# Jittor/JNeRF

Measured on NVIDIA H100. Metric: ngp_lego_train_rays_per_s, higher is better.
Workload: dtype f16

## Files before the change

include/ngp_b200.h:

```cpp
#ifndef NGP_B200_H
#define NGP_B200_H
#include <stdint.h>
#ifdef __cplusplus
extern "C" {
#endif

#define NGP_F32 0
#define NGP_F16 1
#define NGP_N_LEVELS 16
#define NGP_LEVEL_BYTES 32

const char* ngp_last_error(void);
int ngp_version(void);
int ngp_sm_count(void);
int ngp_debug_timeout_flag(void);

int ngp_hash_offsets(double aabb_scale, int n_levels, int base_resolution, int log2_hashmap_size,
                     uint32_t* offsets_out_host, double* per_level_scale_out);
int ngp_hash_level_table(void* stream, const uint32_t* offsets_host, int n_levels, uint32_t base_resolution,
                         float log2_per_level_scale, void* levels_dev);
int ngp_hash_level_table_primes(void* stream, const uint32_t* offsets_host, int n_levels, uint32_t base_resolution,
                                float log2_per_level_scale, void* levels_dev, uint32_t prime0, uint32_t prime1, uint32_t prime2);

int ngp_hash_fwd(void* stream, uint32_t n, const float* x, const void* grid, int dtype, const void* levels_dev, void* out);
// ... 59 lines not shown
                        const uint32_t* numsteps, uint32_t cascades, float* rgb_out, float* alpha_out);
int ngp_composite_loss_bwd(void* stream, uint32_t n_rays, uint32_t n_elements, const void* net_out, const float* coords,
                           const uint32_t* numsteps_in, const uint32_t* numsteps_compacted, const float* bg,
                           const float* target, float huber_delta, const float* density_grid_mean, uint32_t cascades,
                           float* rgb_out, float* loss_out, void* dnet_out, float reg_scale);

int ngp_render_workspace_bytes(uint32_t n_rays, uint32_t capacity, uint64_t* layout_out);
int ngp_render_init(void* stream, uint32_t n_rays, uint32_t capacity, void* workspace, float aabb_lo, float aabb_hi, const float* rays_o,
                    const float* rays_d, float cone_angle, float near_distance, uint32_t cascades, int const_dt, uint64_t rng_state,
                    uint64_t rng_inc, uint32_t jitter_tile, float* rgb_out, float* alpha_out, uint32_t* n_samples_out, uint32_t* n_alive_host);
int ngp_render_march_round(void* stream, uint32_t n_rays, uint32_t capacity, void* workspace, uint32_t n_alive, uint32_t k_steps, float aabb_lo,
                           float aabb_hi, const float* rays_o, const float* rays_d, const uint8_t* bitfield, float cone_angle, uint32_t cascades,
                           int const_dt);
int ngp_render_composite_round(void* stream, uint32_t n_rays, uint32_t capacity, void* workspace, uint32_t n_alive, uint32_t k_steps,
                               float min_transmittance, uint32_t cascades, float* rgb_out, float* alpha_out, uint32_t* n_samples_out,
                               uint32_t* n_alive_host);

int ngp_grid_mark_untrained(void* stream, uint32_t n_elements, float* grid, uint32_t n_images, const float* focal_lengths,
                            const float* xforms, int res_x, int res_y);
int ngp_grid_generate_samples(void* stream, uint32_t n_elements, uint64_t rng_state, uint64_t rng_inc, const uint32_t* step_dev,
                              float aabb_lo, float aabb_hi, const float* grid_in, float* positions_out, uint32_t* indices_out,
                              uint32_t n_cascades, float thresh);
int ngp_grid_splat(void* stream, uint32_t n, const uint32_t* indices, const void* mlp_out, int dtype, float* grid_tmp);
int ngp_grid_ema(void* stream, uint32_t n_elements, float decay, float* grid, const float* grid_tmp);
int ngp_grid_update_bitfield(void* stream, const float* grid, float* mean_out, uint8_t* bitfield, uint32_t cascades);

int ngp_adam_ema(void* stream, uint64_t n, void* param, int param_dtype, void* grad, int grad_dtype, float grad_scale,
                 float* m, float* v, float* master, float lr, float beta1, float beta2, float eps, uint32_t step,
                 float ema_decay, int zero_grad);
int ngp_train_sweep(void* stream, uint64_t n_entries, void* table, float* m, float* v, float* master, void* fx, const float* w_part,
                    uint32_t bwd_rows, void* w_density, float* wd_m, float* wd_v, float* wd_master, void* w_rgb, float* wr_m,
                    float* wr_v, float* wr_master, float lr, float beta1, float beta2, float eps, uint32_t step, float ema_decay);

int ngp_dp_exchange_step(void* stream, int world, int rank, uint64_t slice_len, uint32_t n_w, void* const* peer_table,
                         void* const* peer_table_grad, float* const* peer_w_grad, uint32_t* const* peer_flags, uint32_t epoch, float* m,
                         float* v, float* master, void* w_param, float* w_m, float* w_v, float* w_master, float grad_scale, float lr,
                         float beta1, float beta2, float eps, uint32_t step, float ema_decay);
int ngp_dp_exchange_wait(void* stream, int world, const uint32_t* my_flags, uint32_t epoch);
int ngp_ipc_export(const void* dev_ptr, uint8_t* handle64, uint64_t* offset);
int ngp_ipc_open(const uint8_t* handle64, uint64_t offset, void** dev_ptr);
int ngp_ipc_close(void* dev_ptr, uint64_t offset);

int ngp_raygen(void* stream, uint32_t n, const uint32_t* pix_index, uint32_t W, uint32_t H, const float* xforms,
               const float* focal, const float* principal, uint32_t* img_id_out, float* rays_o, float* rays_d);

int ngp_prepare_batch(void* stream, uint32_t n, const uint32_t* pix_index, uint32_t W, uint32_t H, const float* xforms,
                      const float* focal, const float* principal, const void* images_rgba, int image_is_u8, const float* bg,
// ... 30 lines not shown
```

jnerf_b200/csrc/grid_update.cu:

```cuda
#include "ngp_common.cuh"

namespace {

__global__ void mark_untrained_kernel(uint32_t n_elements, float* __restrict__ grid, uint32_t n_images, const float* __restrict__ focal,
                                      const float* __restrict__ xforms, float half_resx, float half_resy) {
    const uint32_t i = blockIdx.x * blockDim.x + threadIdx.x;
    if (i >= n_elements) return;
    const uint32_t level = i / NERF_GRID_N, pos_idx = i % NERF_GRID_N;
    const uint32_t x = morton3D_invert(pos_idx >> 0), y = morton3D_invert(pos_idx >> 1), z = morton3D_invert(pos_idx >> 2);
    const float sc = scalbnf(1.0f, (int)level);
    const float p[3] = {(((float)x + 0.5f) / NERF_GRIDSIZE - 0.5f) * sc + 0.5f, (((float)y + 0.5f) / NERF_GRIDSIZE - 0.5f) * sc + 0.5f,
                        (((float)z + 0.5f) / NERF_GRIDSIZE - 0.5f) * sc + 0.5f};
    const float voxel_radius = 0.5f * 1.73205080757f * sc / NERF_GRIDSIZE;
    int count = 0;
    for (uint32_t j = 0; j < n_images; ++j) {
        const float* m = xforms + 12 * j;
        const float pl[3] = {p[0] - __ldg(m + 9), p[1] - __ldg(m + 10), p[2] - __ldg(m + 11)};
        const float cx = pl[0] * __ldg(m + 0) + (pl[1] * __ldg(m + 1) + pl[2] * __ldg(m + 2));
        const float cy = pl[0] * __ldg(m + 3) + (pl[1] * __ldg(m + 4) + pl[2] * __ldg(m + 5));
        const float cz = pl[0] * __ldg(m + 6) + (pl[1] * __ldg(m + 7) + pl[2] * __ldg(m + 8));
        if (cz > 0.f) {
            if (fabsf(cx) - voxel_radius < cz / __ldg(focal + 2 * j) * half_resx && fabsf(cy) - voxel_radius < cz / __ldg(focal + 2 * j + 1) * half_resy) {
                count++;
                break;
// ... 26 lines not shown
                        (((float)z + r2) / NERF_GRIDSIZE - 0.5f) * sc + 0.5f};
    positions[3 * (size_t)i] = (p[0] - lo) / diag;
    positions[3 * (size_t)i + 1] = (p[1] - lo) / diag;
    positions[3 * (size_t)i + 2] = (p[2] - lo) / diag;
    indices[i] = idx;
}

template <typename T>
__global__ void splat_kernel(uint32_t n, const uint32_t* __restrict__ indices, const T* __restrict__ mlp_out, float* __restrict__ grid_tmp) {
    const uint32_t i = blockIdx.x * blockDim.x + threadIdx.x;
    if (i >= n) return;
    const float mlp = __expf((float)mlp_out[i]);
    const float thick = mlp * (1.73205080757f / 1024.0f);
    atomicMax(reinterpret_cast<uint32_t*>(grid_tmp) + indices[i], __float_as_uint(thick));
}

__global__ void ema_kernel(uint32_t n, float decay, float* __restrict__ grid, const float* __restrict__ grid_tmp) {
    const uint32_t i = blockIdx.x * blockDim.x + threadIdx.x;
    if (i >= n) return;
    const float prev = grid[i];
    grid[i] = (prev < 0.f) ? prev : fmaxf(prev * decay, grid_tmp[i]);
}

constexpr int MEAN_BLOCKS = 256;
__global__ void __launch_bounds__(256) mean_partial_kernel(const float* __restrict__ grid, float* __restrict__ partial) {
    __shared__ float s[256];
    float acc = 0.f;
    const uint32_t per_block = NERF_GRID_N / MEAN_BLOCKS;
    const float* g = grid + (size_t)blockIdx.x * per_block;
    for (uint32_t k = threadIdx.x; k < per_block; k += 256) acc += fmaxf(g[k], 0.f) / NERF_GRID_N;
    s[threadIdx.x] = acc;
    __syncthreads();
    for (int off = 128; off > 0; off >>= 1) {
        if ((int)threadIdx.x < off) s[threadIdx.x] += s[threadIdx.x + off];
        __syncthreads();
    }
    if (threadIdx.x == 0) partial[blockIdx.x] = s[0];
}
__global__ void __launch_bounds__(256) mean_final_kernel(const float* __restrict__ partial, float* __restrict__ mean) {
    __shared__ float s[256];
    s[threadIdx.x] = partial[threadIdx.x];
    __syncthreads();
    for (int off = 128; off > 0; off >>= 1) {
        if ((int)threadIdx.x < off) s[threadIdx.x] += s[threadIdx.x + off];
        __syncthreads();
    }
// ... 6 lines not shown
    const float m = *mean;
    const float thresh = 0.01f < m ? 0.01f : m;
    const float4 a = reinterpret_cast<const float4*>(grid)[2 * (size_t)i], b = reinterpret_cast<const float4*>(grid)[2 * (size_t)i + 1];
    uint8_t v = 0;
    v |= a.x > thresh ? 1 : 0; v |= a.y > thresh ? 2 : 0; v |= a.z > thresh ? 4 : 0; v |= a.w > thresh ? 8 : 0;
    v |= b.x > thresh ? 16 : 0; v |= b.y > thresh ? 32 : 0; v |= b.z > thresh ? 64 : 0; v |= b.w > thresh ? 128 : 0;
    bits[i] = v;
}
__global__ void bitfield_max_pool_kernel(uint32_t n, const uint8_t* __restrict__ prev, uint8_t* __restrict__ next) {
    const uint32_t i = blockIdx.x * blockDim.x + threadIdx.x;
    if (i >= n) return;
    const uint2 p = reinterpret_cast<const uint2*>(prev)[i];
    uint8_t bits = 0;
#pragma unroll
    for (int j = 0; j < 4; ++j) {
        bits |= ((p.x >> (8 * j)) & 0xFF) ? (uint8_t)(1 << j) : 0;
        bits |= ((p.y >> (8 * j)) & 0xFF) ? (uint8_t)(1 << (4 + j)) : 0;
    }
    const uint32_t x = morton3D_invert(i >> 0) + NERF_GRIDSIZE / 8, y = morton3D_invert(i >> 1) + NERF_GRIDSIZE / 8,
                   z = morton3D_invert(i >> 2) + NERF_GRIDSIZE / 8;
    next[morton3D(x, y, z)] |= bits;
}

float* g_mean_partial = nullptr;

}

extern "C" {

int ngp_grid_mark_untrained(void* stream, uint32_t n_elements, float* grid, uint32_t n_images, const float* focal_lengths, const float* xforms,
                            int res_x, int res_y) {
    if (n_elements == 0) return 0;
    mark_untrained_kernel<<<(n_elements + 127) / 128, 128, 0, (cudaStream_t)stream>>>(n_elements, grid, n_images, focal_lengths, xforms,
                                                                                     res_x * 0.5f, res_y * 0.5f);
    NGP_LAUNCH_CHECK();
    return 0;
}

int ngp_grid_generate_samples(void* stream, uint32_t n_elements, uint64_t rng_state, uint64_t rng_inc, const uint32_t* step_dev, float aabb_lo,
                              float aabb_hi, const float* grid_in, float* positions_out, uint32_t* indices_out, uint32_t n_cascades, float thresh) {
    if (n_elements == 0) return 0;
    generate_samples_kernel<<<(n_elements + 127) / 128, 128, 0, (cudaStream_t)stream>>>(n_elements, rng_state, rng_inc, step_dev, aabb_lo, aabb_hi,
                                                                                       grid_in, positions_out, indices_out, n_cascades, thresh);
    NGP_LAUNCH_CHECK();
    return 0;
}

int ngp_grid_splat(void* stream, uint32_t n, const uint32_t* indices, const void* mlp_out, int dtype, float* grid_tmp) {
    if (n == 0) return 0;
    if (dtype == 1) splat_kernel<__half><<<(n + 127) / 128, 128, 0, (cudaStream_t)stream>>>(n, indices, (const __half*)mlp_out, grid_tmp);
    else if (dtype == 0) splat_kernel<float><<<(n + 127) / 128, 128, 0, (cudaStream_t)stream>>>(n, indices, (const float*)mlp_out, grid_tmp);
    else NGP_REQUIRE(false, "ngp_grid_splat: bad dtype");
    NGP_LAUNCH_CHECK();
    return 0;
}

int ngp_grid_ema(void* stream, uint32_t n_elements, float decay, float* grid, const float* grid_tmp) {
    if (n_elements == 0) return 0;
    ema_kernel<<<(n_elements + 255) / 256, 256, 0, (cudaStream_t)stream>>>(n_elements, decay, grid, grid_tmp);
    NGP_LAUNCH_CHECK();
    return 0;
}

int ngp_grid_update_bitfield(void* stream, const float* grid, float* mean_out, uint8_t* bitfield, uint32_t cascades) {
    NGP_REQUIRE(cascades >= 1 && cascades <= 8, "ngp_grid_update_bitfield: cascades out of range");
    NGP_REQUIRE(((size_t)grid) % 16 == 0, "Can only reduce_sum on 16-byte aligned memory.");
    cudaStream_t s = (cudaStream_t)stream;
    if (!g_mean_partial) NGP_CHECK_CUDA(cudaMalloc(&g_mean_partial, MEAN_BLOCKS * sizeof(float)));
    mean_partial_kernel<<<MEAN_BLOCKS, 256, 0, s>>>(grid, g_mean_partial);
    mean_final_kernel<<<1, 256, 0, s>>>(g_mean_partial, mean_out);
    const uint32_t n = NERF_GRID_N / 8 * cascades;
    grid_to_bitfield_kernel<<<(n + 127) / 128, 128, 0, s>>>(n, grid, bitfield, mean_out);
    for (uint32_t level = 1; level < cascades; ++level) {
        bitfield_max_pool_kernel<<<(NERF_GRID_N / 64 + 127) / 128, 128, 0, s>>>(NERF_GRID_N / 64, bitfield + (size_t)NERF_GRID_N * (level - 1) / 8,
                                                                                bitfield + (size_t)NERF_GRID_N * level / 8);
    }
    NGP_LAUNCH_CHECK();
    return 0;
}

}
```

jnerf_b200/lib.py:

```python
import ctypes as C
import os

HERE = os.path.dirname(os.path.abspath(__file__))
LIB_PATH = os.environ.get("NGP_B200_LIB") or os.path.join(HERE, "libngp_b200.so")

_vp, _u32, _u64, _i64, _f32, _i32, _f64 = C.c_void_p, C.c_uint32, C.c_uint64, C.c_int64, C.c_float, C.c_int, C.c_double

SIGNATURES = {
    "ngp_last_error": (C.c_char_p, []),
    "ngp_version": (_i32, []),
    "ngp_sm_count": (_i32, []),
    "ngp_debug_timeout_flag": (_i32, []),
    "ngp_hash_offsets": (_i32, [_f64, _i32, _i32, _i32, _vp, _vp]),
    "ngp_hash_level_table": (_i32, [_vp, _vp, _i32, _u32, _f32, _vp]),
    "ngp_hash_level_table_primes": (_i32, [_vp, _vp, _i32, _u32, _f32, _vp, _u32, _u32, _u32]),
    "ngp_hash_fwd": (_i32, [_vp, _u32, _vp, _vp, _i32, _vp, _vp]),
    "ngp_hash_bwd": (_i32, [_vp, _u32, _vp, _vp, _i32, _vp, _vp, _u64]),
    "ngp_sh_fwd": (_i32, [_vp, _u32, _vp, _i32, _vp]),
    "ngp_mlp_fwd": (_i32, [_vp, _vp, _vp, _vp, _vp, _u32, _u32]),
    "ngp_mlp_bwd": (_i32, [_vp, _vp, _vp, _vp, _vp, _vp, _vp, _vp, _u32, _u32, _u32]),
    "ngp_mlp_bwd_dgrad": (_i32, [_vp, _vp, _vp, _vp, _vp, _vp, _u32, _u32]),
    "ngp_mlp_param_count": (_i32, [_u32]),
    "ngp_network_fwd": (_i32, [_vp, _u32, _vp, _vp, _vp, _vp, _vp, _vp, _vp, _vp]),
    "ngp_network_bwd": (_i32, [_vp, _u32, _vp, _vp, _vp, _vp, _vp, _vp, _vp, _vp, _vp, _vp]),
# ... 6 lines not shown
    "ngp_nerf_density": (_i32, [_vp, _u32, _vp, _vp, _vp]),
    "ngp_nerf_bwd": (_i32, [_vp, _u32, _vp, _vp, _vp, _vp, _vp, _vp]),
    "ngp_mesh_workspace_bytes": (_i32, [_u32, _u64, _u64, _vp]),
    "ngp_density_lattice": (_i32, [_vp, _u32, _vp, _vp, _vp, _vp]),
    "ngp_marching_cubes": (_i32, [_vp, _u32, _vp, _f32, _vp, _vp, _u64, _vp, _u64, _vp]),
    "ngp_mesh_largest_component": (_i32, [_vp, _u64, _u64, _vp, _vp, _vp, _vp, _vp, _vp]),
    "ngp_mesh_vertex_normals": (_i32, [_vp, _u64, _u64, _vp, _vp, _vp, _vp]),
    "ngp_mesh_smooth_workspace_bytes": (_i32, [_u32, _u32, _vp]),
    "ngp_mesh_smooth": (_i32, [_vp, _u32, _vp, _u32, _u32, _vp, _u64, _vp, _vp]),
    "ngp_render_workspace_bytes": (_i32, [_u32, _u32, _vp]),
    "ngp_render_init": (_i32, [_vp, _u32, _u32, _vp, _f32, _f32, _vp, _vp, _f32, _f32, _u32, _i32, _u64, _u64, _u32, _vp, _vp, _vp, _vp]),
    "ngp_render_march_round": (_i32, [_vp, _u32, _u32, _vp, _u32, _u32, _f32, _f32, _vp, _vp, _vp, _f32, _u32, _i32]),
    "ngp_render_composite_round": (_i32, [_vp, _u32, _u32, _vp, _u32, _u32, _f32, _u32, _vp, _vp, _vp, _vp]),
    "ngp_march_workspace_bytes": (_u64, [_u32]),
    "ngp_march": (_i32, [_vp, _u32, _f32, _f32, _u32, _vp, _vp, _vp, _f32, _f32, _u32, _i32, _u64, _u64, _vp, _vp, _vp, _vp, _vp]),
    "ngp_compact": (_i32, [_vp, _u32, _u32, _vp, _vp, _vp, _vp, _vp, _i32]),
    "ngp_composite_fwd": (_i32, [_vp, _u32, _vp, _i32, _vp, _vp, _vp, _vp, _u32, _vp]),
    "ngp_composite_bwd": (_i32, [_vp, _u32, _u32, _vp, _i32, _vp, _vp, _vp, _vp, _vp, _u32, _vp]),
    "ngp_composite_infer": (_i32, [_vp, _u32, _vp, _i32, _vp, _vp, _u32, _vp, _vp]),
    "ngp_composite_loss_bwd": (_i32, [_vp, _u32, _u32, _vp, _vp, _vp, _vp, _vp, _vp, _f32, _vp, _u32, _vp, _vp, _vp, _f32]),
    "ngp_grid_mark_untrained": (_i32, [_vp, _u32, _vp, _u32, _vp, _vp, _i32, _i32]),
    "ngp_grid_generate_samples": (_i32, [_vp, _u32, _u64, _u64, _vp, _f32, _f32, _vp, _vp, _vp, _u32, _f32]),
    "ngp_grid_splat": (_i32, [_vp, _u32, _vp, _vp, _i32, _vp]),
    "ngp_grid_ema": (_i32, [_vp, _u32, _f32, _vp, _vp]),
    "ngp_grid_update_bitfield": (_i32, [_vp, _vp, _vp, _vp, _u32]),
    "ngp_adam_ema": (_i32, [_vp, _u64, _vp, _i32, _vp, _i32, _f32, _vp, _vp, _vp, _f32, _f32, _f32, _f32, _u32, _f32, _i32]),
    "ngp_train_sweep": (_i32, [_vp, _u64, _vp, _vp, _vp, _vp, _vp, _vp, _u32, _vp, _vp, _vp, _vp, _vp, _vp, _vp, _vp, _f32, _f32, _f32, _f32, _u32,
                               _f32]),
    "ngp_train_sweep_dev": (_i32, [_vp, _u64, _vp, _vp, _vp, _vp, _vp, _vp, _u32, _vp, _vp, _vp, _vp, _vp, _vp, _vp, _vp, _vp]),
    "ngp_dp_exchange_step": (_i32, [_vp, _i32, _i32, _u64, _u32, _vp, _vp, _vp, _vp, _u32, _vp, _vp, _vp, _vp, _vp, _vp, _vp, _f32, _f32, _f32,
                                    _f32, _f32, _u32, _f32]),
    "ngp_dp_exchange_wait": (_i32, [_vp, _i32, _vp, _u32]),
    "ngp_ipc_export": (_i32, [_vp, _vp, _vp]),
    "ngp_ipc_open": (_i32, [_vp, _u64, _vp]),
    "ngp_ipc_close": (_i32, [_vp, _u64]),
    "ngp_raygen": (_i32, [_vp, _u32, _vp, _u32, _u32, _vp, _vp, _vp, _vp, _vp, _vp]),
    "ngp_prepare_batch": (_i32, [_vp, _u32, _vp, _u32, _u32, _vp, _vp, _vp, _vp, _i32, _vp, _vp, _vp, _vp, _vp]),
    "ngp_blend_target": (_i32, [_vp, _u32, _vp, _vp, _vp]),
    "ngp_step_state_bytes": (_u64, []),
    "ngp_step_state_set": (_i32, [_vp, _vp, _u64, _u64, _u32, _u32, _f32, _f32, _f32, _f32, _f32, _f32]),
    "ngp_step_state_tick": (_i32, [_vp, _vp, _u32, _f32, _f32, _f32, _f32, _f32, _f32]),
    "ngp_prepare_batch_dev": (_i32, [_vp, _u32, _vp, _vp, _u32, _u32, _u32, _vp, _vp, _vp, _vp, _i32, _vp, _vp, _vp, _vp, _vp]),
    "ngp_march_dev": (_i32, [_vp, _u32, _f32, _f32, _u32, _vp, _vp, _vp, _f32, _f32, _u32, _i32, _vp, _u32, _vp, _vp, _vp, _vp, _vp]),
    "ngp_adam_ema_dev": (_i32, [_vp, _u64, _vp, _i32, _vp, _i32, _vp, _vp, _vp, _vp, _i32]),
    "ngp_pcg32_seed": (None, [_u64, _u64, _vp]),
    "ngp_pcg32_advance": (None, [_vp, _i64]),
}

KERNELS_PER_CALL = {
    "ngp_hash_level_table": 1, "ngp_hash_level_table_primes": 1, "ngp_hash_fwd": 1, "ngp_hash_bwd": 1, "ngp_sh_fwd": 1, "ngp_mlp_fwd": 1, "ngp_mlp_bwd": 1, "ngp_mlp_bwd_dgrad": 1,
    "ngp_network_fwd": 1, "ngp_network_bwd": 1, "ngp_network_bwd_fx": 1, "ngp_train_sweep": 1, "ngp_train_sweep_dev": 1, "ngp_density_fwd": 1, "ngp_march": 3, "ngp_compact": 1, "ngp_composite_fwd": 1,
    "ngp_composite_bwd": 1, "ngp_composite_infer": 1, "ngp_composite_loss_bwd": 1, "ngp_grid_mark_untrained": 1,
    "ngp_grid_generate_samples": 1, "ngp_grid_splat": 1, "ngp_grid_ema": 1, "ngp_grid_update_bitfield": 7, "ngp_adam_ema": 1, "ngp_dp_exchange_step": 1, "ngp_dp_exchange_wait": 1, "ngp_raygen": 1, "ngp_prepare_batch": 1,
    "ngp_blend_target": 1, "ngp_step_state_set": 1, "ngp_step_state_tick": 1, "ngp_prepare_batch_dev": 1, "ngp_march_dev": 3, "ngp_adam_ema_dev": 1,
    "ngp_density_lattice": 1, "ngp_marching_cubes": 3, "ngp_mesh_largest_component": 18, "ngp_mesh_vertex_normals": 7,
    "ngp_render_init": 3, "ngp_render_march_round": 3, "ngp_render_composite_round": 3,
    "ngp_nerf_fwd": 1, "ngp_nerf_density": 1, "ngp_nerf_bwd": 3,
}
launch_count = 0
_lib = None


class NgpError(RuntimeError):
    pass


def load():
    global _lib
    if _lib is None:
        if not os.path.exists(LIB_PATH):
            raise NgpError(f"{LIB_PATH} is missing: build it with `python jnerf_b200/build.py` (nvcc, sm_90a). "
                           "There is no CPU fallback.")
        lib = C.CDLL(LIB_PATH)
        for name, (res, args) in SIGNATURES.items():
            fn = getattr(lib, name)
            fn.restype = res
# ... 14 lines not shown
```

jnerf_b200/ops.py:

```python
import numpy as np
import torch

from . import lib

F32, F16 = 0, 1


def _dt(t):
    if t.dtype == torch.float16:
        return F16
    if t.dtype == torch.float32:
        return F32
    raise TypeError(f"unsupported dtype {t.dtype}")


def _p(t):
    if t is None:
        return None
    assert t.is_cuda and t.is_contiguous(), "device-resident contiguous tensor required"
    return t.data_ptr()


_raw_stream, _raw_device = getattr(torch._C, "_cuda_getCurrentRawStream", None), getattr(torch._C, "_cuda_getDevice", None)

# ... 340 lines not shown
    if loss is None:
        loss = torch.empty(R, dtype=torch.float32, device=dev)
    lib.call("ngp_composite_loss_bwd", _stream(), R, net.shape[0], _p(net), _p(coords), _p(numsteps_in), _p(numsteps_c), _p(bg), _p(target),
             float(delta), _p(mean), cascades, _p(rgb), _p(loss), _p(dnet), float(reg_scale))
    return rgb, loss, dnet


def grid_mark_untrained(grid, focal, xforms, res):
    lib.call("ngp_grid_mark_untrained", _stream(), grid.numel(), _p(grid), xforms.shape[0], _p(focal), _p(xforms), int(res[0]), int(res[1]))


def grid_generate_samples(n, rng, step_dev, aabb, grid, n_cascades, thresh):
    pos = torch.empty((n, 3), dtype=torch.float32, device=grid.device)
    idx = torch.empty(n, dtype=torch.int32, device=grid.device)
    lib.call("ngp_grid_generate_samples", _stream(), n, int(rng[0]), int(rng[1]), _p(step_dev), float(aabb[0]), float(aabb[1]), _p(grid), _p(pos),
             _p(idx), n_cascades, float(thresh))
    return pos, idx


def grid_splat(indices, mlp_out, grid_tmp):
    lib.call("ngp_grid_splat", _stream(), indices.numel(), _p(indices), _p(mlp_out), _dt(mlp_out), _p(grid_tmp))


def grid_ema(grid, grid_tmp, decay=0.95):
    lib.call("ngp_grid_ema", _stream(), grid.numel(), float(decay), _p(grid), _p(grid_tmp))


def grid_update_bitfield(grid, mean, bitfield, cascades=5):
    lib.call("ngp_grid_update_bitfield", _stream(), _p(grid), _p(mean), _p(bitfield), cascades)


def adam_ema(param, grad, m, v, master, lr, step, beta1=0.9, beta2=0.99, eps=1e-15, ema_decay=0.95, grad_scale=1.0, zero_grad=True):
    lib.call("ngp_adam_ema", _stream(), param.numel(), _p(param), _dt(param), _p(grad), _dt(grad), float(grad_scale), _p(m), _p(v), _p(master),
             float(lr), float(beta1), float(beta2), float(eps), int(step), float(ema_decay), int(zero_grad))


def raygen(pix, W, H, xforms, focal, principal):
    n = pix.numel()
    dev = pix.device
    img = torch.empty(n, dtype=torch.int32, device=dev)
    o = torch.empty((n, 3), dtype=torch.float32, device=dev)
    d = torch.empty((n, 3), dtype=torch.float32, device=dev)
    lib.call("ngp_raygen", _stream(), n, _p(pix), W, H, _p(xforms), _p(focal), _p(principal), _p(img), _p(o), _p(d))
    return img, o, d


def prepare_batch(pix, W, H, xforms, focal, principal, images, bg):
    n = pix.numel()
# ... 86 lines not shown
```

jnerf_b200/plugin/sampler.py:

```python
import math

import numpy as np
import torch

from .. import ops
from ..utils.config import get_cfg
from ..utils.registry import SAMPLERS
from .module import Module


class _CalcRgbFn(torch.autograd.Function):

    @staticmethod
    def forward(ctx, network_output, coords, numsteps, numsteps_compacted, bg, mean, cascades):
        network_output = network_output.contiguous()
        rgb = ops.composite_fwd(network_output, coords, numsteps, numsteps_compacted, bg, cascades)
        ctx.save_for_backward(network_output, coords, numsteps_compacted, rgb, mean)
        ctx.cascades = cascades
        return rgb

    @staticmethod
    def backward(ctx, grad_x):
        net, coords, ns_c, rgb, mean = ctx.saved_tensors
        dnet = ops.composite_bwd(net, coords, ns_c, grad_x.contiguous(), rgb, mean, ctx.cascades)
# ... 21 lines not shown
        self.NERF_MIN_OPTICAL_THICKNESS = 0.01
        self.MAX_STEP = 1024
        self.background_color = self.cfg.background_color
        self.n_images = self.dataset.n_images
        self.image_resolutions = self.dataset.resolution
        self.aabb_range = self.dataset.aabb_range
        max_aabb_scale = 1 << (self.NERF_CASCADES - 1)
        if self.dataset.aabb_scale > max_aabb_scale:
            self.NERF_CASCADES = math.ceil(math.log2(self.dataset.aabb_scale)) + 1
        self.max_cascade = 0
        while (1 << self.max_cascade) < self.dataset.aabb_scale:
            self.max_cascade += 1
        dev = "cuda"
        G3 = self.NERF_GRIDSIZE ** 3
        self.density_grid_decay = 0.95
        self.density_n_elements = self.NERF_CASCADES * G3
        self.density_grid = torch.zeros(self.density_n_elements, dtype=torch.float32, device=dev)
        self.density_grid_tmp = torch.zeros(self.density_n_elements, dtype=torch.float32, device=dev)
        self.density_grid_bitfield = torch.zeros(self.density_n_elements // 8, dtype=torch.uint8, device=dev)
        self.density_grid_mean = torch.zeros(1, dtype=torch.float32, device=dev)
        self.density_grid_ema_step = torch.zeros(1, dtype=torch.int32, device=dev)
        self.measured_batch_size = torch.zeros(1, dtype=torch.int32, device=dev)
        self.rng = ops.pcg32_seed(1337)
        self.max_samples = self.cfg.n_rays_per_batch * self.MAX_STEP
        self._coords_raw = torch.zeros((self.max_samples, 7), dtype=torch.float32, device=dev)
        self._march_ws_rays = 0
        self._march_ws = None
        self._ensure_march_ws(max(2 * self.n_rays_per_batch, 8192))
        self.dp_group = None
        self._coords = None
        self._rays_numsteps = None
        self._rays_numsteps_compacted = None
        self._counters_compacted = None

    def _ensure_march_ws(self, n_rays):
        if n_rays > self._march_ws_rays:
            self._march_ws = None
            self._march_ws_rays = int(n_rays)
            self._march_ws = torch.empty(int(ops.lib.load().ngp_march_workspace_bytes(self._march_ws_rays)) + 16, dtype=torch.uint8, device="cuda")

    def sample(self, img_ids, rays_o, rays_d, rgb_target=None, is_training=False, ray_index_offset=0):
        if is_training:
            if self.cfg.m_training_step % self.update_den_freq == 0:
                self.update_density_grid()
            self._rays_numsteps, self._rays_numsteps_compacted, self._counters_compacted, self._coords = self.sample_front(
                rays_o, rays_d, self._coords_raw, ray_index_offset)
# ... 38 lines not shown
        self._rays_numsteps = rays_numsteps
        self._coords = coords[:cap]
        self._rays_numsteps_compacted = ns_c
        self._counters_compacted = cnt_c

    @property
    def coords_compacted(self):
        return self._coords

    @property
    def n_samples_dev(self):
        return self._counters_compacted[0:1]

    def rays2rgb(self, network_outputs, training_background_color=None, inference=False):
        assert network_outputs.shape[0] == self._coords.shape[0]
        if inference:
            return ops.composite_infer(network_outputs.contiguous(), self._coords, self._rays_numsteps, self.NERF_CASCADES)
        bg = training_background_color
        if bg is None:
            bg = torch.tensor(self.background_color, dtype=torch.float32, device="cuda").expand(self._rays_numsteps.shape[0], 3).contiguous()
        return _CalcRgbFn.apply(network_outputs, self._coords, self._rays_numsteps, self._rays_numsteps_compacted, bg.contiguous(),
                                self.density_grid_mean, self.NERF_CASCADES)

    def update_density_grid_nerf(self, decay, n_uniform, n_nonuniform):
        if self.cfg.m_training_step == 0:
            self.density_grid.zero_()
            ops.grid_mark_untrained(self.density_grid, self.dataset.focal_lengths, self.dataset.transforms_gpu, self.image_resolutions)
        self.density_grid_tmp.zero_()
        parts_p, parts_i = [], []
        for n, thresh in ((n_uniform, -0.01), (n_nonuniform, self.NERF_MIN_OPTICAL_THICKNESS)):
            if n == 0:
                continue
            p, i = ops.grid_generate_samples(n, self.rng, self.density_grid_ema_step, self.aabb_range, self.density_grid, self.max_cascade + 1, thresh)
            ops.pcg32_advance(self.rng)
            parts_p.append(p)
            parts_i.append(i)
        pos = torch.cat(parts_p) if len(parts_p) > 1 else parts_p[0]
        idx = torch.cat(parts_i) if len(parts_i) > 1 else parts_i[0]
        with torch.no_grad():
            bs = self.update_block_size
            res = [self.model.density(pos[i:i + bs]) for i in range(0, pos.shape[0], bs)]
            mlp_out = (torch.cat(res, 0) if len(res) > 1 else res[0]).reshape(-1).contiguous()
        ops.grid_splat(idx, mlp_out, self.density_grid_tmp)
        ops.grid_ema(self.density_grid, self.density_grid_tmp, decay)
        self.density_grid_ema_step += 1
        ops.grid_update_bitfield(self.density_grid, self.density_grid_mean, self.density_grid_bitfield, self.NERF_CASCADES)

    def update_density_grid(self):
        G3 = self.NERF_GRIDSIZE ** 3
        n_cascades = self.max_cascade + 1
        if self.cfg.m_training_step < 256:
            self.update_density_grid_nerf(self.density_grid_decay, G3 * n_cascades, 0)
        else:
            self.update_density_grid_nerf(self.density_grid_decay, G3 * n_cascades // 4, G3 * n_cascades // 4)

    def update_batch_rays(self, measured_total=None):
        from .. import dp
        W = 1
        if measured_total is not None:
            W = self.dp_group[1] if self.dp_group is not None else 1
            self.n_rays_per_batch = max(dp.adapt_rays_per_batch(self.n_rays_per_batch * W, measured_total / 16, self.target_batch_size * W) // W, 1)
            self.dataset.batch_size = self.n_rays_per_batch
            return
        if self.dp_group is not None:
            W = self.dp_group[1]
            dp.global_sum_count(self.measured_batch_size, self.dp_group[0], W)
        measured = self.measured_batch_size.item() / 16
        self.n_rays_per_batch = max(dp.adapt_rays_per_batch(self.n_rays_per_batch * W, measured, self.target_batch_size * W) // W, 1)
        self.measured_batch_size.zero_()
        self.dataset.batch_size = self.n_rays_per_batch

    def state_dict(self, *args, **kwargs):
        return {"density_grid": self.density_grid, "density_grid_bitfield": self.density_grid_bitfield, "density_grid_mean": self.density_grid_mean,
                "density_grid_ema_step": self.density_grid_ema_step, "n_rays_per_batch": self.n_rays_per_batch,
                "rng": torch.from_numpy(self.rng.astype(np.int64))}

    def load_state_dict(self, sd, *args, **kwargs):
# ... 8 lines not shown
```

jnerf_b200/runner.py:

```python
import contextlib
import os

import numpy as np
import torch

from . import dp, ops
from .plugin import losses as L
from .utils.config import get_cfg
from .utils.registry import DATASETS, LOSSES, NETWORKS, OPTIMS, SAMPLERS, build_from_cfg


class Runner:
    def __init__(self, rank=0, world_size=1, process_group=None):
        self.cfg = get_cfg()
        cfg = self.cfg
        self.rank, self.world_size, self.pg = rank, world_size, process_group
        self.dataset = {"train": build_from_cfg(cfg.dataset.train, DATASETS)}
        cfg.dataset_obj = self.dataset["train"]
        self.dataset["val"] = build_from_cfg(cfg.dataset.val, DATASETS) if cfg.dataset.val else self.dataset["train"]
        self.dataset["test"] = None
        self.model = build_from_cfg(cfg.model, NETWORKS)
        cfg.model_obj = self.model
        self.sampler = build_from_cfg(cfg.sampler, SAMPLERS)
        cfg.sampler_obj = self.sampler
# ... 35 lines not shown
        n_w = m.density_mlp.con_weights.numel() + m.rgb_mlp.con_weights.numel()
        self.w_grad = torch.zeros(n_w + 8, dtype=torch.float32, device=dev)
        self.dwd = self.w_grad[:m.density_mlp.con_weights.numel()]
        self.dwr = self.w_grad[m.density_mlp.con_weights.numel():n_w]
        self.net_out = torch.zeros((cap, 4), dtype=torch.float16, device=dev)
        self.enc = torch.empty((cap, 32), dtype=torch.float16, device=dev)
        self.dnet = torch.zeros((cap, 4), dtype=torch.float16, device=dev)
        self.last_loss = None
        self.last_rgb = None
        self._fx = self._w_part = None
        if self.world_size == 1 and ops.network_bwd is ops._network_bwd:
            self._fx, self._w_part = ops.network_bwd_scratch(m.pos_encoder.levels, device=dev)
        if self.world_size == 1:
            self._dev_state = ops.step_state_new()
            self._dev_expect = None
            self._graphs, self._graph_seen, self._graph_pool, self._cap_stream = {}, {}, None, None
            self._graphs_enabled = os.environ.get("NGP_GRAPHS", "0") == "1" and torch.cuda.is_available() and hasattr(torch.cuda, "CUDAGraph")
            self.graph_replays = 0
            self._graph_after = int(os.environ.get("NGP_GRAPH_AFTER", "20"))
        if os.environ.get("NGP_PIPELINE", "1") == "1" and not getattr(self, "_graphs_enabled", False):
            raw = self.sampler._coords_raw
            self._pipe = dict(stream=torch.cuda.Stream(), coords=[torch.zeros_like(raw), torch.zeros_like(raw)], made=0, pending=None, at="front",
                              mid=torch.cuda.Event(), back_done=[torch.cuda.Event(), torch.cuda.Event()], prefetched=0, aux=torch.cuda.Stream(),
                              aux_done=torch.cuda.Event(), main=None)
        if self.world_size > 1:
            self._init_sharded_table()

    def _init_sharded_table(self):
        import os
        g = self.model.pos_encoder.m_grid
        m = self.model
        n, W = g.numel(), self.world_size
        mode = os.environ.get("NGP_DP_EXCHANGE", "auto")
        assert mode in ("auto", "p2p", "nccl")
        self.dp_mode = "p2p" if mode == "p2p" or (mode == "auto" and dp.peer_exchange_available(W)) else "nccl"
        P = dp.padded_len(n, W)
        nd, nr = m.density_mlp.con_weights.numel(), m.rgb_mlp.con_weights.numel()
        if self.dp_mode == "p2p":
            try:
                self._arena = dp.PeerArena(n, nd + nr, W, self.rank, self.pg)
            except RuntimeError as e:
                if mode == "p2p":
                    raise
                if self.rank == 0:
                    print(f"[jnerf_b200] peer-memory exchange unavailable ({e}); using the NCCL exchange", flush=True)
                self.dp_mode = "nccl"
        if self.dp_mode == "p2p":
# ... 177 lines not shown
        ops.pcg32_advance(s.rng)
        dec.advance_lr()
        adam.n_step += 1
        self.ema_optimizer.steps += 1
        self._dev_expect = (int(s.rng[0]), int(s.rng[1]), start + R, adam.n_step, lr_next)
        if i % s.update_den_freq == s.update_den_freq - 1:
            s.update_batch_rays()
        cfg.m_training_step = i + 1
        return loss

    def _front(self, step, batch, prefetch):
        P, s = self._pipe, self.sampler
        slot = P["made"] & 1
        main = P["main"] if P["main"] is not None else torch.cuda.current_stream()
        side = P["stream"]
        if prefetch:
            side.wait_event(P["mid"])
        (side if prefetch else main).wait_event(P["back_done"][slot])
        with (torch.cuda.stream(side) if prefetch else contextlib.nullcontext()):
            rng_before = s.rng.copy()
            if step % s.update_den_freq == 0:
                assert not prefetch
                self._table_ready()
                s.update_density_grid()
            img_ids, rays_o, rays_d, bg, target = self._batch(batch)
            numsteps, ns_c, cnt_c, coords = s.sample_front(rays_o, rays_d, P["coords"][slot],
                                                           ray_index_offset=dp.shard_range(rays_o.shape[0], self.rank)[0])
            done = torch.cuda.Event()
            done.record(side if prefetch else main)
        P["made"] += 1
        P["prefetched"] += int(prefetch)
        return dict(step=step, src=batch, slot=slot, bg=bg, target=target, numsteps=numsteps, ns_c=ns_c, cnt_c=cnt_c, coords=coords, done=done,
                    rng_before=rng_before, rays=(img_ids, rays_o, rays_d), side=prefetch)

    def _adapt_ray_batch(self, F):
        P, s = self._pipe, self.sampler
        side = P["stream"]
        if P.get("count_host") is None:
            P["count_host"], P["count_ev"] = torch.zeros(1, dtype=torch.int32).pin_memory(), torch.cuda.Event()
        side.wait_event(F["done"])
        with torch.cuda.stream(side):
            if self.world_size > 1:
                dp.global_sum_count(s.measured_batch_size, self.pg, self.world_size)
            P["count_host"].copy_(s.measured_batch_size, non_blocking=True)
            s.measured_batch_size.zero_()
            P["count_ev"].record(side)
        P["count_ev"].synchronize()
# ... 9 lines not shown
        cfg, s, P = self.cfg, self.sampler, self._pipe
        i = cfg.m_training_step
        main = P["main"] = torch.cuda.current_stream()
        F, P["pending"] = P["pending"], None
        if F is not None and (F["step"] != i or F["src"] is not batch):
            main.wait_event(F["done"])
            F = None
        if F is None:
            F = self._front(i, batch, prefetch=False)
        elif F["side"]:
            main.wait_event(F["done"])
        P["mid"].record(main)
        s.__dict__.update(_rays_numsteps=F["numsteps"], _rays_numsteps_compacted=F["ns_c"], _counters_compacted=F["cnt_c"], _coords=F["coords"])
        rgb, loss = self._net_pass(F["bg"], F["target"], zero_on=(P["aux"], P["aux_done"]))
        self._optimizer_tail()
        P["back_done"][F["slot"]].record(main)
        self.last_loss, self.last_rgb = loss, rgb
        cfg.m_training_step = i + 1
        self._pipe_last = F
        if i % s.update_den_freq == s.update_den_freq - 1:
            self._adapt_ray_batch(F)
        if (i + 1) % s.update_den_freq != 0 and (batch is None or next_batch is not None):
            P["pending"] = self._front(i + 1, next_batch if batch is not None else None, prefetch=True)
        return loss

    def train_step(self, batch=None, next_batch=None):
        if self._pipe is not None:
            return self._train_step_pipe(batch, next_batch)
        if batch is None and self._dev_state is not None:
            return self._train_step_dev()
        cfg, s = self.cfg, self.sampler
        i = cfg.m_training_step
        img_ids, rays_o, rays_d, bg, target = self._batch(batch)
        if i % s.update_den_freq == 0:
            self._table_ready()
        s.sample(img_ids, rays_o, rays_d, is_training=True,
                 ray_index_offset=dp.shard_range(rays_o.shape[0], self.rank)[0])
        rgb, loss = self._net_pass(bg, target)
        self._optimizer_tail()
        self.last_loss, self.last_rgb = loss, rgb
        cfg.m_training_step = i + 1
        return loss

    def train_step_host(self, batch, next_batch=None):
        st = self._host_stage
        if st is None:
# ... 395 lines not shown
        ds = self.dataset[dataset_mode]
        n = ds.n_images if max_images is None else min(max_images, ds.n_images)
        tot = 0.0
        for k in range(n):
            img, tar = self.render_img(dataset_mode, k)
            tot += float(L.mse2psnr(L.img2mse(img, tar)).item())
        return tot / n

    def save_ckpt(self, path):
        adam = self.optimizer._nested_optimizer
        self._table_ready()
        nested = adam.state_dict()
        if self.world_size > 1:
            k = [id(s.p) for s in adam.state].index(id(self.model.pos_encoder.m_grid))
            full = self._gather_table_state()
            for key, t in zip(("m", "v", "master"), full):
                nested[key] = list(nested[key])
                nested[key][k] = t
            if self.rank != 0:
                return
        sampler_state = self.sampler.state_dict()
        if self._pipe is not None and self._pipe["pending"] is not None:
            sampler_state["rng"] = torch.from_numpy(self._pipe["pending"]["rng_before"].astype(np.int64))
        ck = {"global_step": self.cfg.m_training_step, "model": self.model.state_dict(), "sampler": sampler_state,
              "optimizer": self.optimizer.state_dict(), "nested_optimizer": nested, "ema_optimizer": self.ema_optimizer.state_dict()}
        if str(path).endswith(".pkl") and not hasattr(getattr(self.model, "density_mlp", None), "con_weights"):
            raise NotImplementedError(f"the .pkl interchange format is written for the fused-MLP parameter layout (con_weights) of "
                                      f"NGPNetworks; save {type(self.model).__name__} to a .pt path")
        if str(path).endswith(".pkl"):
            from .utils import ckpt_compat as cc
            dec = self.optimizer
            ref = cc.native_to_reference(
                ck, adam_hyper=dict(lr=adam.lr, eps=adam.eps, betas=tuple(adam.betas)),
                expdecay_hyper=dict(base_lr=dec.base_lr, decay_start=dec.decay_start, decay_interval=dec.decay_interval, decay_base=dec.decay_base,
                                    decay_end=dec.decay_end),
                param_dtype=np.float16 if self.model.pos_encoder.m_grid.dtype == torch.float16 else np.float32)
            cc.write_reference_ckpt(ref, path)
            return
        torch.save(ck, path)

    def load_ckpt(self, path):
        self._table_ready()
        if self._pipe is not None:
            self._sync_front()
            self._pipe["pending"] = None
        if self.world_size > 1:
            import torch.distributed as dist
            dist.barrier(group=self.pg)
        if str(path).endswith(".pkl") and not hasattr(getattr(self.model, "density_mlp", None), "con_weights"):
            raise NotImplementedError("the .pkl interchange format carries the fused-MLP parameter layout; load a .pt checkpoint instead")
        if str(path).endswith(".pkl"):
            from .utils import ckpt_compat as cc
            ck = cc.load_native_from_reference_file(path, self.model.pos_encoder.m_grid.numel(), "cuda",
                                                    {k: v.dtype for k, v in self.model.state_dict().items()})
        else:
            ck = torch.load(path, map_location="cuda", weights_only=True)
        self.cfg.m_training_step = self.start = ck["global_step"]
        self.model.load_state_dict(ck["model"])
        self.sampler.load_state_dict(ck["sampler"])
        self.optimizer.load_state_dict(ck["optimizer"])
        nested = ck["nested_optimizer"]
        if self.world_size > 1:
            adam = self.optimizer._nested_optimizer
            k = [id(s.p) for s in adam.state].index(id(self.model.pos_encoder.m_grid))
            self._scatter_table_state(nested["m"][k], nested["v"][k], nested["master"][k])
            st = self._st[id(self.model.pos_encoder.m_grid)]
            nested = dict(nested, **{key: [t if j != k else getattr(st, key) for j, t in enumerate(nested[key])] for key in ("m", "v", "master")})
            self._slice_param.copy_(self._table[self._lo:self._hi])
# ... 56 lines not shown
```

Before: 3.210 million.

## Overlap density-grid sample generation on side stream, sort samples, fuse EMA with clear

Density-grid update samples are now drawn on the side stream during the preceding step and consumed at the update step, overlapping sample generation with training work. Samples are bucket-sorted by cell index (counting sort with scan) so that density MLP queries and splat atomics hit nearby cells together. The EMA kernel is fused with clearing grid_tmp, which removes the separate zero_ pass and skips writes to unchanged grid entries. This adds a sort pass, extra stream synchronisation and RNG-state bookkeeping for checkpoints.

```diff
diff --git a/include/ngp_b200.h b/include/ngp_b200.h
--- a/include/ngp_b200.h
+++ b/include/ngp_b200.h
@@ -105,7 +105,11 @@
                               float aabb_lo, float aabb_hi, const float* grid_in, float* positions_out, uint32_t* indices_out,
                               uint32_t n_cascades, float thresh);
 int ngp_grid_splat(void* stream, uint32_t n, const uint32_t* indices, const void* mlp_out, int dtype, float* grid_tmp);
+int ngp_grid_sort_workspace_bytes(uint32_t n_cells, uint64_t* bytes_out);
+int ngp_grid_sort_samples(void* stream, uint32_t n, const float* positions, const uint32_t* indices, uint32_t n_cells, void* workspace,
+                          uint64_t workspace_bytes, float* positions_out, uint32_t* indices_out);
 int ngp_grid_ema(void* stream, uint32_t n_elements, float decay, float* grid, const float* grid_tmp);
+int ngp_grid_ema_clear(void* stream, uint32_t n_elements, uint32_t n_sampled, float decay, float* grid, float* grid_tmp);
 int ngp_grid_update_bitfield(void* stream, const float* grid, float* mean_out, uint8_t* bitfield, uint32_t cascades);
 
 int ngp_adam_ema(void* stream, uint64_t n, void* param, int param_dtype, void* grad, int grad_dtype, float grad_scale,
diff --git a/jnerf_b200/csrc/grid_update.cu b/jnerf_b200/csrc/grid_update.cu
--- a/jnerf_b200/csrc/grid_update.cu
+++ b/jnerf_b200/csrc/grid_update.cu
@@ -1,4 +1,5 @@
 #include "ngp_common.cuh"
+#include "mesh_scan.cuh"
 
 namespace {
 
@@ -72,6 +73,19 @@
     grid[i] = (prev < 0.f) ? prev : fmaxf(prev * decay, grid_tmp[i]);
 }
 
+__global__ void ema_clear_kernel(uint32_t n, uint32_t n_sampled, float decay, float* __restrict__ grid, float* __restrict__ grid_tmp) {
+    const uint32_t i = blockIdx.x * blockDim.x + threadIdx.x;
+    if (i >= n) return;
+    const float prev = grid[i];
+    float t = 0.f;
+    if (i < n_sampled) {
+        t = grid_tmp[i];
+        if (__float_as_uint(t) != 0u) grid_tmp[i] = 0.f;
+    }
+    const float next = (prev < 0.f) ? prev : fmaxf(prev * decay, t);
+    if (__float_as_uint(next) != __float_as_uint(prev)) grid[i] = next;
+}
+
 constexpr int MEAN_BLOCKS = 256;
 __global__ void __launch_bounds__(256) mean_partial_kernel(const float* __restrict__ grid, float* __restrict__ partial) {
     __shared__ float s[256];
@@ -124,6 +138,33 @@
     next[morton3D(x, y, z)] |= bits;
 }
 
+constexpr uint32_t SORT_SHIFT = 3;
+
+__global__ void sort_count_kernel(uint32_t n, const uint32_t* __restrict__ indices, uint32_t n_keys, uint32_t* __restrict__ count) {
+    const uint32_t i = blockIdx.x * blockDim.x + threadIdx.x;
+    if (i >= n) return;
+    const uint32_t key = indices[i] >> SORT_SHIFT;
+    if (key < n_keys) atomicAdd(count + key, 1u);
+}
+
+__global__ void sort_scatter_kernel(uint32_t n, const float* __restrict__ positions, const uint32_t* __restrict__ indices, uint32_t n_keys,
+                                    uint32_t* __restrict__ cursor, float* __restrict__ positions_out, uint32_t* __restrict__ indices_out) {
+    const uint32_t i = blockIdx.x * blockDim.x + threadIdx.x;
+    if (i >= n) return;
+    const uint32_t idx = indices[i];
+    if ((idx >> SORT_SHIFT) >= n_keys) return;
+    const uint32_t d = atomicAdd(cursor + (idx >> SORT_SHIFT), 1u);
+    positions_out[3 * (size_t)d] = positions[3 * (size_t)i];
+    positions_out[3 * (size_t)d + 1] = positions[3 * (size_t)i + 1];
+    positions_out[3 * (size_t)d + 2] = positions[3 * (size_t)i + 2];
+    indices_out[d] = idx;
+}
+
+uint64_t sort_workspace_bytes(uint32_t n_cells) {
+    const uint64_t n_keys = n_cells >> SORT_SHIFT;
+    return 4 * (n_keys + (n_keys + ngp_mesh::SCAN_BLOCK - 1) / ngp_mesh::SCAN_BLOCK + 1);
+}
+
 float* g_mean_partial = nullptr;
 
 }
@@ -157,9 +198,46 @@
     return 0;
 }
 
+int ngp_grid_sort_workspace_bytes(uint32_t n_cells, uint64_t* bytes_out) {
+    NGP_REQUIRE(bytes_out, "ngp_grid_sort_workspace_bytes: bytes_out is NULL");
+    *bytes_out = sort_workspace_bytes(n_cells);
+    return 0;
+}
+
+int ngp_grid_sort_samples(void* stream, uint32_t n, const float* positions, const uint32_t* indices, uint32_t n_cells, void* workspace,
+                          uint64_t workspace_bytes, float* positions_out, uint32_t* indices_out) {
+    NGP_REQUIRE(n_cells > 0 && n_cells % NERF_GRID_N == 0 && n_cells / NERF_GRID_N <= 8,
+                "ngp_grid_sort_samples: n_cells must be 1 to 8 cascades of 128^3 cells");
+    NGP_REQUIRE(workspace && workspace_bytes >= sort_workspace_bytes(n_cells), "ngp_grid_sort_samples: workspace too small");
+    if (n == 0) return 0;
+    NGP_REQUIRE(positions && indices && positions_out && indices_out, "ngp_grid_sort_samples: NULL buffer");
+    NGP_REQUIRE(positions != positions_out && indices != indices_out, "ngp_grid_sort_samples: cannot sort in place");
+    cudaStream_t s = (cudaStream_t)stream;
+    const uint32_t n_keys = n_cells >> SORT_SHIFT;
+    uint32_t* count = (uint32_t*)workspace;
+    uint32_t* bsum = count + n_keys;
+    NGP_CHECK_CUDA(cudaMemsetAsync(count, 0, 4ull * n_keys, s));
+    sort_count_kernel<<<(n + 255) / 256, 256, 0, s>>>(n, indices, n_keys, count);
+    NGP_LAUNCH_CHECK();
+    const uint32_t n_bsum = (n_keys + ngp_mesh::SCAN_BLOCK - 1) / ngp_mesh::SCAN_BLOCK;
+    if (int rc = ngp_mesh::scan_u32(s, count, n_keys, bsum, bsum + n_bsum)) return rc;
+    sort_scatter_kernel<<<(n + 255) / 256, 256, 0, s>>>(n, positions, indices, n_keys, count, positions_out, indices_out);
+    NGP_LAUNCH_CHECK();
+    return 0;
+}
+
 int ngp_grid_ema(void* stream, uint32_t n_elements, float decay, float* grid, const float* grid_tmp) {
     if (n_elements == 0) return 0;
     ema_kernel<<<(n_elements + 255) / 256, 256, 0, (cudaStream_t)stream>>>(n_elements, decay, grid, grid_tmp);
+    NGP_LAUNCH_CHECK();
+    return 0;
+}
+
+int ngp_grid_ema_clear(void* stream, uint32_t n_elements, uint32_t n_sampled, float decay, float* grid, float* grid_tmp) {
+    NGP_REQUIRE(n_sampled <= n_elements, "ngp_grid_ema_clear: n_sampled exceeds n_elements");
+    if (n_elements == 0) return 0;
+    NGP_REQUIRE(grid && grid_tmp, "ngp_grid_ema_clear: NULL buffer");
+    ema_clear_kernel<<<(n_elements + 255) / 256, 256, 0, (cudaStream_t)stream>>>(n_elements, n_sampled, decay, grid, grid_tmp);
     NGP_LAUNCH_CHECK();
     return 0;
 }
diff --git a/jnerf_b200/lib.py b/jnerf_b200/lib.py
--- a/jnerf_b200/lib.py
+++ b/jnerf_b200/lib.py
@@ -52,7 +52,10 @@
     "ngp_grid_mark_untrained": (_i32, [_vp, _u32, _vp, _u32, _vp, _vp, _i32, _i32]),
     "ngp_grid_generate_samples": (_i32, [_vp, _u32, _u64, _u64, _vp, _f32, _f32, _vp, _vp, _vp, _u32, _f32]),
     "ngp_grid_splat": (_i32, [_vp, _u32, _vp, _vp, _i32, _vp]),
+    "ngp_grid_sort_workspace_bytes": (_i32, [_u32, _vp]),
+    "ngp_grid_sort_samples": (_i32, [_vp, _u32, _vp, _vp, _u32, _vp, _u64, _vp, _vp]),
     "ngp_grid_ema": (_i32, [_vp, _u32, _f32, _vp, _vp]),
+    "ngp_grid_ema_clear": (_i32, [_vp, _u32, _u32, _f32, _vp, _vp]),
     "ngp_grid_update_bitfield": (_i32, [_vp, _vp, _vp, _vp, _u32]),
     "ngp_adam_ema": (_i32, [_vp, _u64, _vp, _i32, _vp, _i32, _f32, _vp, _vp, _vp, _f32, _f32, _f32, _f32, _u32, _f32, _i32]),
     "ngp_train_sweep": (_i32, [_vp, _u64, _vp, _vp, _vp, _vp, _vp, _vp, _u32, _vp, _vp, _vp, _vp, _vp, _vp, _vp, _vp, _f32, _f32, _f32, _f32, _u32,
@@ -81,7 +84,7 @@
     "ngp_hash_level_table": 1, "ngp_hash_level_table_primes": 1, "ngp_hash_fwd": 1, "ngp_hash_bwd": 1, "ngp_sh_fwd": 1, "ngp_mlp_fwd": 1, "ngp_mlp_bwd": 1, "ngp_mlp_bwd_dgrad": 1,
     "ngp_network_fwd": 1, "ngp_network_bwd": 1, "ngp_network_bwd_fx": 1, "ngp_train_sweep": 1, "ngp_train_sweep_dev": 1, "ngp_density_fwd": 1, "ngp_march": 3, "ngp_compact": 1, "ngp_composite_fwd": 1,
     "ngp_composite_bwd": 1, "ngp_composite_infer": 1, "ngp_composite_loss_bwd": 1, "ngp_grid_mark_untrained": 1,
-    "ngp_grid_generate_samples": 1, "ngp_grid_splat": 1, "ngp_grid_ema": 1, "ngp_grid_update_bitfield": 7, "ngp_adam_ema": 1, "ngp_dp_exchange_step": 1, "ngp_dp_exchange_wait": 1, "ngp_raygen": 1, "ngp_prepare_batch": 1,
+    "ngp_grid_generate_samples": 1, "ngp_grid_splat": 1, "ngp_grid_sort_samples": 5, "ngp_grid_ema": 1, "ngp_grid_ema_clear": 1, "ngp_grid_update_bitfield": 7, "ngp_adam_ema": 1, "ngp_dp_exchange_step": 1, "ngp_dp_exchange_wait": 1, "ngp_raygen": 1, "ngp_prepare_batch": 1,
     "ngp_blend_target": 1, "ngp_step_state_set": 1, "ngp_step_state_tick": 1, "ngp_prepare_batch_dev": 1, "ngp_march_dev": 3, "ngp_adam_ema_dev": 1,
     "ngp_density_lattice": 1, "ngp_marching_cubes": 3, "ngp_mesh_largest_component": 18, "ngp_mesh_vertex_normals": 7,
     "ngp_render_init": 3, "ngp_render_march_round": 3, "ngp_render_composite_round": 3,
diff --git a/jnerf_b200/ops.py b/jnerf_b200/ops.py
--- a/jnerf_b200/ops.py
+++ b/jnerf_b200/ops.py
@@ -386,8 +386,29 @@
     lib.call("ngp_grid_splat", _stream(), indices.numel(), _p(indices), _p(mlp_out), _dt(mlp_out), _p(grid_tmp))
 
 
+_grid_splat = grid_splat
+
+
+def grid_sort_workspace(n_cells, device="cuda"):
+    b = np.zeros(1, np.uint64)
+    lib.call("ngp_grid_sort_workspace_bytes", int(n_cells), b.ctypes.data)
+    return torch.empty(int(b[0]), dtype=torch.uint8, device=device)
+
+
+def grid_sort_samples(pos, idx, n_cells, workspace):
+    assert pos.shape == (idx.numel(), 3) and pos.dtype == torch.float32 and idx.dtype == torch.int32
+    pos_out, idx_out = torch.empty_like(pos), torch.empty_like(idx)
+    lib.call("ngp_grid_sort_samples", _stream(), idx.numel(), _p(pos), _p(idx), int(n_cells), _p(workspace), workspace.numel(), _p(pos_out),
+             _p(idx_out))
+    return pos_out, idx_out
+
+
 def grid_ema(grid, grid_tmp, decay=0.95):
     lib.call("ngp_grid_ema", _stream(), grid.numel(), float(decay), _p(grid), _p(grid_tmp))
+
+
+def grid_ema_clear(grid, grid_tmp, n_sampled, decay=0.95):
+    lib.call("ngp_grid_ema_clear", _stream(), grid.numel(), int(n_sampled), float(decay), _p(grid), _p(grid_tmp))
 
 
 def grid_update_bitfield(grid, mean, bitfield, cascades=5):
diff --git a/jnerf_b200/plugin/sampler.py b/jnerf_b200/plugin/sampler.py
--- a/jnerf_b200/plugin/sampler.py
+++ b/jnerf_b200/plugin/sampler.py
@@ -67,6 +67,8 @@
         self.density_grid_ema_step = torch.zeros(1, dtype=torch.int32, device=dev)
         self.measured_batch_size = torch.zeros(1, dtype=torch.int32, device=dev)
         self.rng = ops.pcg32_seed(1337)
+        self._grid_sort_ws = None
+        self._grid_tmp_clear = True
         self.max_samples = self.cfg.n_rays_per_batch * self.MAX_STEP
         self._coords_raw = torch.zeros((self.max_samples, 7), dtype=torch.float32, device=dev)
         self._march_ws_rays = 0
@@ -151,11 +153,28 @@
         return _CalcRgbFn.apply(network_outputs, self._coords, self._rays_numsteps, self._rays_numsteps_compacted, bg.contiguous(),
                                 self.density_grid_mean, self.NERF_CASCADES)
 
-    def update_density_grid_nerf(self, decay, n_uniform, n_nonuniform):
+    def update_density_grid_nerf(self, decay, n_uniform, n_nonuniform, samples=None):
         if self.cfg.m_training_step == 0:
             self.density_grid.zero_()
             ops.grid_mark_untrained(self.density_grid, self.dataset.focal_lengths, self.dataset.transforms_gpu, self.image_resolutions)
-        self.density_grid_tmp.zero_()
+        lib_ops = self.lib_grid_ops
+        if not (lib_ops and self._grid_tmp_clear):
+            self.density_grid_tmp.zero_()
+        pos, idx = self._draw_grid_samples(n_uniform, n_nonuniform) if samples is None else samples
+        with torch.no_grad():
+            bs = self.update_block_size
+            res = [self.model.density(pos[i:i + bs]) for i in range(0, pos.shape[0], bs)]
+            mlp_out = (torch.cat(res, 0) if len(res) > 1 else res[0]).reshape(-1).contiguous()
+        ops.grid_splat(idx, mlp_out, self.density_grid_tmp)
+        if lib_ops:
+            ops.grid_ema_clear(self.density_grid, self.density_grid_tmp, (self.max_cascade + 1) * self.NERF_GRIDSIZE ** 3, decay)
+        else:
+            ops.grid_ema(self.density_grid, self.density_grid_tmp, decay)
+        self._grid_tmp_clear = lib_ops
+        self.density_grid_ema_step += 1
+        ops.grid_update_bitfield(self.density_grid, self.density_grid_mean, self.density_grid_bitfield, self.NERF_CASCADES)
+
+    def _draw_grid_samples(self, n_uniform, n_nonuniform):
         parts_p, parts_i = [], []
         for n, thresh in ((n_uniform, -0.01), (n_nonuniform, self.NERF_MIN_OPTICAL_THICKNESS)):
             if n == 0:
@@ -166,22 +185,30 @@
             parts_i.append(i)
         pos = torch.cat(parts_p) if len(parts_p) > 1 else parts_p[0]
         idx = torch.cat(parts_i) if len(parts_i) > 1 else parts_i[0]
-        with torch.no_grad():
-            bs = self.update_block_size
-            res = [self.model.density(pos[i:i + bs]) for i in range(0, pos.shape[0], bs)]
-            mlp_out = (torch.cat(res, 0) if len(res) > 1 else res[0]).reshape(-1).contiguous()
-        ops.grid_splat(idx, mlp_out, self.density_grid_tmp)
-        ops.grid_ema(self.density_grid, self.density_grid_tmp, decay)
-        self.density_grid_ema_step += 1
-        ops.grid_update_bitfield(self.density_grid, self.density_grid_mean, self.density_grid_bitfield, self.NERF_CASCADES)
-
-    def update_density_grid(self):
+        if self.lib_grid_ops:
+            n_cells = (self.max_cascade + 1) * self.NERF_GRIDSIZE ** 3
+            if self._grid_sort_ws is None:
+                self._grid_sort_ws = ops.grid_sort_workspace(n_cells)
+            pos, idx = ops.grid_sort_samples(pos, idx, n_cells, self._grid_sort_ws)
+        return pos, idx
+
+    @property
+    def lib_grid_ops(self):
+        return ops.grid_splat is ops._grid_splat
+
+    def _grid_sample_counts(self):
         G3 = self.NERF_GRIDSIZE ** 3
         n_cascades = self.max_cascade + 1
         if self.cfg.m_training_step < 256:
-            self.update_density_grid_nerf(self.density_grid_decay, G3 * n_cascades, 0)
-        else:
-            self.update_density_grid_nerf(self.density_grid_decay, G3 * n_cascades // 4, G3 * n_cascades // 4)
+            return G3 * n_cascades, 0
+        return G3 * n_cascades // 4, G3 * n_cascades // 4
+
+    def grid_samples(self):
+        assert self.cfg.m_training_step != 0
+        return self._draw_grid_samples(*self._grid_sample_counts())
+
+    def update_density_grid(self, samples=None):
+        self.update_density_grid_nerf(self.density_grid_decay, *self._grid_sample_counts(), samples=samples)
 
     def update_batch_rays(self, measured_total=None):
         from .. import dp
diff --git a/jnerf_b200/runner.py b/jnerf_b200/runner.py
--- a/jnerf_b200/runner.py
+++ b/jnerf_b200/runner.py
@@ -81,7 +81,7 @@
             raw = self.sampler._coords_raw
             self._pipe = dict(stream=torch.cuda.Stream(), coords=[torch.zeros_like(raw), torch.zeros_like(raw)], made=0, pending=None, at="front",
                               mid=torch.cuda.Event(), back_done=[torch.cuda.Event(), torch.cuda.Event()], prefetched=0, aux=torch.cuda.Stream(),
-                              aux_done=torch.cuda.Event(), main=None)
+                              aux_done=torch.cuda.Event(), main=None, grid=None)
         if self.world_size > 1:
             self._init_sharded_table()
 
@@ -305,7 +305,15 @@
             if step % s.update_den_freq == 0:
                 assert not prefetch
                 self._table_ready()
-                s.update_density_grid()
+                G, P["grid"] = P["grid"], None
+                if G is not None:
+                    main.wait_event(G["done"])
+                if G is not None and G["step"] == step:
+                    for t in G["samples"]:
+                        t.record_stream(main)
+                    s.update_density_grid(samples=G["samples"])
+                else:
+                    s.update_density_grid()
             img_ids, rays_o, rays_d, bg, target = self._batch(batch)
             numsteps, ns_c, cnt_c, coords = s.sample_front(rays_o, rays_d, P["coords"][slot],
                                                            ray_index_offset=dp.shard_range(rays_o.shape[0], self.rank)[0])
@@ -361,6 +369,15 @@
             self._adapt_ray_batch(F)
         if (i + 1) % s.update_den_freq != 0 and (batch is None or next_batch is not None):
             P["pending"] = self._front(i + 1, next_batch if batch is not None else None, prefetch=True)
+        elif (i + 1) % s.update_den_freq == 0 and s.lib_grid_ops:
+            side = P["stream"]
+            side.wait_event(P["mid"])
+            with torch.cuda.stream(side):
+                rng_before = s.rng.copy()
+                samples = s.grid_samples()
+                done = torch.cuda.Event()
+                done.record(side)
+            P["grid"] = dict(step=i + 1, samples=samples, done=done, rng_before=rng_before)
         return loss
 
     def train_step(self, batch=None, next_batch=None):
@@ -802,6 +819,8 @@
         sampler_state = self.sampler.state_dict()
         if self._pipe is not None and self._pipe["pending"] is not None:
             sampler_state["rng"] = torch.from_numpy(self._pipe["pending"]["rng_before"].astype(np.int64))
+        elif self._pipe is not None and self._pipe["grid"] is not None:
+            sampler_state["rng"] = torch.from_numpy(self._pipe["grid"]["rng_before"].astype(np.int64))
         ck = {"global_step": self.cfg.m_training_step, "model": self.model.state_dict(), "sampler": sampler_state,
               "optimizer": self.optimizer.state_dict(), "nested_optimizer": nested, "ema_optimizer": self.ema_optimizer.state_dict()}
         if str(path).endswith(".pkl") and not hasattr(getattr(self.model, "density_mlp", None), "con_weights"):
@@ -824,6 +843,9 @@
         if self._pipe is not None:
             self._sync_front()
             self._pipe["pending"] = None
+            if self._pipe["grid"] is not None:
+                torch.cuda.current_stream().wait_event(self._pipe["grid"]["done"])
+                self._pipe["grid"] = None
         if self.world_size > 1:
             import torch.distributed as dist
             dist.barrier(group=self.pg)
```

After: 3.223 million, median of 6. No clear change (+0.4%).
